# CrawlScript/tf_geometric

Measured on NVIDIA H100. Metric: edges/sec GCN+GAT fwd on 2.4M-node/123M-edge synthetic; %HBM roofline, higher is better.
Workload: dtype f32

## Files before the change

### tf_geometric_b200/csrc/gemm_proj.cu

```cuda
#include "common.cuh"
#include <type_traits>

namespace tfgk {
namespace proj {

constexpr int BM = 128;
constexpr int BK = 32;
constexpr int kUN = 128;
constexpr int kThreads = 256;
constexpr int kApitch = BK + 4;
constexpr int kStageBytes = BM * kApitch * 4;
constexpr int kMaxBlocks = 4;
constexpr int kMaxParts = 8;

struct Params {
    const float *A[kMaxParts];
    int64_t lda, part_rows;
    int first_tile;
    int M, K, kpad, nb, tiles_m, n_groups;
    const float *B[kMaxBlocks]; int64_t ldb[kMaxBlocks];
    const float *bias[kMaxBlocks]; int act[kMaxBlocks]; int ncols[kMaxBlocks]; int transb[kMaxBlocks];
    float *C[kMaxBlocks]; int64_t ldc[kMaxBlocks];
};

struct Plan {
    uint32_t kpad, b_bytes, ring_off, stages, total;
    explicit Plan(int K) {
        kpad = (uint32_t)((K + 7) / 8) * 8;
        b_bytes = (uint32_t)kUN * kpad * 4u;
        ring_off = 2u * b_bytes + kUN * 4u;
        const uint32_t budget = 227u * 1024u;
        stages = 0;
        for (uint32_t st = 4; st >= 2; --st)
            if (ring_off + st * kStageBytes <= budget) { stages = st; break; }
        total = ring_off + stages * kStageBytes;
    }
};

__device__ __forceinline__ uint32_t smem_u32(const void *p) { return (uint32_t)__cvta_generic_to_shared(p); }

__device__ __forceinline__ uint32_t w_offset(int n, int k, int kpad) {
    return (uint32_t)(n >> 3) * (uint32_t)(kpad * 32) + (uint32_t)(k >> 2) * 128u + (uint32_t)(n & 7) * 16u + (uint32_t)(k & 3) * 4u;
}

__device__ __forceinline__ uint64_t make_desc(uint32_t saddr, uint32_t sbo_bytes) {
    uint64_t d = 0;
    d |= (uint64_t)((saddr & 0x3FFFFu) >> 4);
    d |= (uint64_t)(128u >> 4) << 16;
    d |= (uint64_t)(sbo_bytes >> 4) << 32;
    return d;
}

__device__ __forceinline__ void split_tf32(float a, uint32_t &hi, uint32_t &lo) {
    asm("cvt.rna.tf32.f32 %0, %1;" : "=r"(hi) : "f"(a));
    lo = __float_as_uint(a - __uint_as_float(hi));
}

__device__ __forceinline__ void cp_async16_zfill(uint32_t dst, const void *src, uint32_t src_bytes) {
    asm volatile("cp.async.cg.shared.global [%0], [%1], 16, %2;" ::"r"(dst), "l"(src), "r"(src_bytes) : "memory");
}

__device__ __forceinline__ void wgmma_fence() { asm volatile("wgmma.fence.sync.aligned;" ::: "memory"); }
__device__ __forceinline__ void wgmma_commit() { asm volatile("wgmma.commit_group.sync.aligned;" ::: "memory"); }
__device__ __forceinline__ void wgmma_wait_all() { asm volatile("wgmma.wait_group.sync.aligned 0;" ::: "memory"); }

__device__ __forceinline__ void wgmma_m64n128k8(float (&d)[64], const uint32_t (&a)[4], uint64_t b_desc, uint32_t accumulate) {
    asm volatile(
        "{\n\t.reg .pred p;\n\t"
        "setp.ne.b32 p, %69, 0;\n\t"
        "wgmma.mma_async.sync.aligned.m64n128k8.f32.tf32.tf32 "
        "{%0, %1, %2, %3, %4, %5, %6, %7, %8, %9, %10, %11, %12, %13, %14, %15, "
        "%16, %17, %18, %19, %20, %21, %22, %23, %24, %25, %26, %27, %28, %29, %30, %31, "
        "%32, %33, %34, %35, %36, %37, %38, %39, %40, %41, %42, %43, %44, %45, %46, %47, "
        "%48, %49, %50, %51, %52, %53, %54, %55, %56, %57, %58, %59, %60, %61, %62, %63}, "
        "{%64, %65, %66, %67}, %68, p, 1, 1;\n\t}"
        : "+f"(d[0]), "+f"(d[1]), "+f"(d[2]), "+f"(d[3]), "+f"(d[4]), "+f"(d[5]), "+f"(d[6]), "+f"(d[7]),
          "+f"(d[8]), "+f"(d[9]), "+f"(d[10]), "+f"(d[11]), "+f"(d[12]), "+f"(d[13]), "+f"(d[14]), "+f"(d[15]),
          "+f"(d[16]), "+f"(d[17]), "+f"(d[18]), "+f"(d[19]), "+f"(d[20]), "+f"(d[21]), "+f"(d[22]), "+f"(d[23]),
          "+f"(d[24]), "+f"(d[25]), "+f"(d[26]), "+f"(d[27]), "+f"(d[28]), "+f"(d[29]), "+f"(d[30]), "+f"(d[31]),
          "+f"(d[32]), "+f"(d[33]), "+f"(d[34]), "+f"(d[35]), "+f"(d[36]), "+f"(d[37]), "+f"(d[38]), "+f"(d[39]),
          "+f"(d[40]), "+f"(d[41]), "+f"(d[42]), "+f"(d[43]), "+f"(d[44]), "+f"(d[45]), "+f"(d[46]), "+f"(d[47]),
          "+f"(d[48]), "+f"(d[49]), "+f"(d[50]), "+f"(d[51]), "+f"(d[52]), "+f"(d[53]), "+f"(d[54]), "+f"(d[55]),
          "+f"(d[56]), "+f"(d[57]), "+f"(d[58]), "+f"(d[59]), "+f"(d[60]), "+f"(d[61]), "+f"(d[62]), "+f"(d[63])
        : "r"(a[0]), "r"(a[1]), "r"(a[2]), "r"(a[3]), "l"(b_desc), "r"(accumulate)
        : "memory");
}

__device__ __forceinline__ int tile_index(const Params &p, int group, int it) {
    int tl = group + it * p.n_groups + p.first_tile;
    return tl >= p.tiles_m ? tl - p.tiles_m : tl;
}

template <int STAGES>
__global__ void __launch_bounds__(kThreads, 1) gemm_proj_kernel(const Params p) {
    extern __shared__ __align__(128) uint8_t smem[];
    const int tid = threadIdx.x, lane = tid & 31, warp = tid >> 5;
    const int cb = blockIdx.x % p.nb, group = blockIdx.x / p.nb;
    const int kpad = p.kpad;
    const uint32_t b_bytes = (uint32_t)kUN * kpad * 4u;
    uint8_t *w_hi = smem, *w_lo = smem + b_bytes;
    float *s_bias = reinterpret_cast<float *>(smem + 2 * b_bytes);
    uint8_t *ring = smem + 2 * b_bytes + kUN * 4;
    const uint32_t ring_addr = smem_u32(ring);

    const int ncols = p.ncols[cb];
    const int my_tiles = group < p.tiles_m ? (p.tiles_m - group + p.n_groups - 1) / p.n_groups : 0;
    const int kb_per_tile = (p.K + BK - 1) / BK;
    const int total = my_tiles * kb_per_tile;

    auto load_stage = [&](int j) {
        if (j < total) {
            const int64_t row0 = (int64_t)tile_index(p, group, j / kb_per_tile) * BM;
            const int part = (int)(row0 / p.part_rows);
            const float *a_tile = p.A[part] + (row0 - (int64_t)part * p.part_rows) * p.lda;
            const int rows = (int)min((int64_t)BM, (int64_t)p.M - row0);
            const int k0 = (j % kb_per_tile) * BK;
            const uint32_t dst0 = ring_addr + (uint32_t)(j % STAGES) * kStageBytes;
            const int ch = tid & 7, gk = k0 + ch * 4;
            const uint32_t bytes = gk < p.K ? (uint32_t)min(16, (p.K - gk) * 4) : 0u;
#pragma unroll
            for (int i = 0; i < (BM * BK / 4) / kThreads; ++i) {
                const int r = (tid >> 3) + i * (kThreads / 8);
                const bool ok = r < rows && bytes != 0;
                cp_async16_zfill(dst0 + (uint32_t)(r * kApitch + ch * 4) * 4u, ok ? a_tile + (int64_t)r * p.lda + gk : p.A[0],
                                 ok ? bytes : 0u);
            }
        }
        asm volatile("cp.async.commit_group;" ::: "memory");
    };

#pragma unroll
    for (int s = 0; s < STAGES - 1; ++s) load_stage(s);

    {
        const float *B = p.B[cb];
        const int64_t ldb = p.ldb[cb];
        const bool tb = p.transb[cb] != 0;
        for (int idx = tid; idx < kUN * kpad; idx += kThreads) {
            int n, k;
            if (tb) { n = idx / kpad; k = idx % kpad; } else { k = idx / kUN; n = idx % kUN; }
            const float w = (n < ncols && k < p.K) ? (tb ? B[(int64_t)n * ldb + k] : B[(int64_t)k * ldb + n]) : 0.0f;
            uint32_t hi, lo;
            split_tf32(w, hi, lo);
            const uint32_t off = w_offset(n, k, kpad);
            *reinterpret_cast<uint32_t *>(w_hi + off) = hi;
            *reinterpret_cast<uint32_t *>(w_lo + off) = lo;
        }
        if (tid < kUN) s_bias[tid] = (p.bias[cb] != nullptr && tid < ncols) ? p.bias[cb][tid] : 0.0f;
    }
    asm volatile("fence.proxy.async.shared::cta;" ::: "memory");
    __syncthreads();

    const uint32_t w_hi_addr = smem_u32(w_hi), w_lo_addr = smem_u32(w_lo), sbo = (uint32_t)kpad * 32u;
    const int frag_row = (warp >> 2) * 64 + (warp & 3) * 16 + (lane >> 2);
    const int frag_col = lane & 3;
    const int act = p.act[cb];
    float *C = p.C[cb];
    const int64_t ldc = p.ldc[cb];
    const bool vec2 = (ldc % 2) == 0 && (reinterpret_cast<uintptr_t>(C) & 7u) == 0;
    float acc[64];
#pragma unroll
    for (int i = 0; i < 64; ++i) acc[i] = 0.0f;

    uint32_t ah[2][BK / 8][4], al[2][BK / 8][4];
    auto stage = [&](auto parity, int j) {
        constexpr int P = decltype(parity)::value;
        asm volatile("cp.async.wait_group %0;" ::"n"(STAGES - 2) : "memory");
        __syncthreads();
        load_stage(j + STAGES - 1);
        const int kb = j % kb_per_tile;
        const float *As = reinterpret_cast<const float *>(ring + (size_t)(j % STAGES) * kStageBytes);
#pragma unroll
        for (int ks = 0; ks < BK / 8; ++ks) {
            const float *a_r0 = As + frag_row * kApitch + ks * 8 + frag_col;
            const float *a_r8 = a_r0 + 8 * kApitch;
            split_tf32(a_r0[0], ah[P][ks][0], al[P][ks][0]);
            split_tf32(a_r8[0], ah[P][ks][1], al[P][ks][1]);
            split_tf32(a_r0[4], ah[P][ks][2], al[P][ks][2]);
            split_tf32(a_r8[4], ah[P][ks][3], al[P][ks][3]);
        }
        wgmma_wait_all();
        wgmma_fence();
#pragma unroll
        for (int ks = 0; ks < BK / 8; ++ks) {
            const int kg = kb * BK + ks * 8;
            if (kg < kpad) {
                const uint32_t koff = (uint32_t)(kg >> 2) * 128u;
                const uint64_t dh = make_desc(w_hi_addr + koff, sbo), dl = make_desc(w_lo_addr + koff, sbo);
                wgmma_m64n128k8(acc, al[P][ks], dh, (kb | ks) != 0);
                wgmma_m64n128k8(acc, ah[P][ks], dl, 1u);
                wgmma_m64n128k8(acc, ah[P][ks], dh, 1u);
            }
        }
        wgmma_commit();
        if (kb == kb_per_tile - 1) {
            wgmma_wait_all();
            const int64_t row0 = (int64_t)tile_index(p, group, j / kb_per_tile) * BM + frag_row;
#pragma unroll
            for (int h = 0; h < 2; ++h) {
                const int64_t row = row0 + 8 * h;
                if (row < p.M) {
                    float *crow = C + row * ldc;
#pragma unroll
                    for (int nb8 = 0; nb8 < kUN / 8; ++nb8) {
                        const int col = nb8 * 8 + 2 * frag_col;
                        const float v0 = apply_act(acc[4 * nb8 + 2 * h] + s_bias[col], act);
                        const float v1 = apply_act(acc[4 * nb8 + 2 * h + 1] + s_bias[col + 1], act);
                        if (vec2 && col + 1 < ncols) {
                            *reinterpret_cast<float2 *>(crow + col) = make_float2(v0, v1);
                        } else {
                            if (col < ncols) crow[col] = v0;
                            if (col + 1 < ncols) crow[col + 1] = v1;
                        }
                    }
                }
            }
        }
    };
    for (int j = 0; j < total; j += 2) {
        stage(std::integral_constant<int, 0>(), j);
        if (j + 1 < total) stage(std::integral_constant<int, 1>(), j + 1);
    }
    wgmma_wait_all();
    asm volatile("cp.async.wait_group 0;" ::: "memory");
}

template <int STAGES>
static int launch(const Params &p, int grid, uint32_t smem_bytes, cudaStream_t st) {
    TFGK_CUDA(ensure_dynamic_smem(gemm_proj_kernel<STAGES>, smem_bytes));
    gemm_proj_kernel<STAGES><<<grid, kThreads, smem_bytes, st>>>(p);
    TFGK_LAUNCH_CHECK();
    return TFGK_OK;
}

}
}

using namespace tfgk;

extern "C" int tfgk_gemm_proj_f32(const float *const *A_parts, int32_t n_parts, int64_t part_rows, int64_t lda,
                                  int32_t M, int32_t K, const tfgk_proj_block *blocks, int32_t n_blocks,
                                  int32_t first_part, int32_t max_ctas, void *stream) {
    TFGK_CHECK_ARG(A_parts != nullptr && blocks != nullptr, "gemm_proj: null argument");
    TFGK_CHECK_ARG(n_parts >= 1 && n_parts <= proj::kMaxParts, "gemm_proj: n_parts=%d not in [1, %d]", n_parts, proj::kMaxParts);
    TFGK_CHECK_ARG(n_blocks >= 1 && n_blocks <= proj::kMaxBlocks, "gemm_proj: n_blocks=%d not in [1, %d]", n_blocks, proj::kMaxBlocks);
    TFGK_CHECK_ARG(M >= 0 && K >= 1, "gemm_proj: bad size (M=%d, K=%d)", M, K);
    TFGK_CHECK_ARG(first_part >= 0 && first_part < n_parts, "gemm_proj: first_part=%d out of range", first_part);
    if (M == 0) return TFGK_OK;
    if (n_parts > 1)
        TFGK_CHECK_ARG(part_rows > 0 && part_rows % proj::BM == 0 && (int64_t)n_parts * part_rows >= M,
                       "gemm_proj: part_rows=%lld must be a positive multiple of %d covering M=%d", (long long)part_rows, proj::BM, M);
    if (K > 512 || (lda % 4) != 0 || lda < K) return TFGK_ERR_UNSUPPORTED;
    proj::Params p;
    for (int i = 0; i < proj::kMaxParts; ++i) {
        p.A[i] = A_parts[i < n_parts ? i : 0];
        if (!aligned16(p.A[i]) || p.A[i] == nullptr) return i < n_parts && A_parts[i] == nullptr
            ? set_error(TFGK_ERR_INVALID_ARGUMENT, "gemm_proj: A part %d is null", i) : TFGK_ERR_UNSUPPORTED;
    }
    p.lda = lda; p.part_rows = n_parts > 1 ? part_rows : (int64_t)1 << 40;
    p.M = M; p.K = K; p.nb = n_blocks;
    p.tiles_m = (int)ceil_div64(M, proj::BM);
    p.first_tile = n_parts > 1 ? (int)((int64_t)first_part * part_rows / proj::BM) : 0;
    if (p.first_tile >= p.tiles_m) p.first_tile = 0;
    for (int b = 0; b < proj::kMaxBlocks; ++b) {
        const tfgk_proj_block &blk = blocks[b < n_blocks ? b : 0];
        if (b < n_blocks) {
            TFGK_CHECK_ARG(blk.B != nullptr && blk.C != nullptr, "gemm_proj: block %d has a null operand", b);
            TFGK_CHECK_ARG(blk.ncols >= 1 && blk.ldb >= (blk.transB ? K : blk.ncols) && blk.ldc >= blk.ncols,
                           "gemm_proj: block %d has bad sizes", b);
            TFGK_CHECK_ARG(blk.act == TFGK_ACT_NONE || blk.act == TFGK_ACT_RELU, "gemm_proj: unknown activation %d", blk.act);
            if (blk.ncols > proj::kUN) return TFGK_ERR_UNSUPPORTED;
        }
        p.B[b] = blk.B; p.ldb[b] = blk.ldb; p.bias[b] = blk.bias; p.act[b] = blk.act; p.ncols[b] = blk.ncols;
        p.transb[b] = blk.transB;
        p.C[b] = blk.C; p.ldc[b] = blk.ldc;
    }
    const proj::Plan L(K);
    if (L.stages == 0) return TFGK_ERR_UNSUPPORTED;
    p.kpad = (int)L.kpad;
    int dev = 0, sms = 0;
    TFGK_CUDA(cudaGetDevice(&dev));
    TFGK_CUDA(cudaDeviceGetAttribute(&sms, cudaDevAttrMultiProcessorCount, dev));
    if (max_ctas > 0 && max_ctas < sms) sms = max_ctas;
    int n_groups = sms / n_blocks;
    if (n_groups < 1) n_groups = 1;
    if (n_groups > p.tiles_m) n_groups = p.tiles_m;
    p.n_groups = n_groups;
    const int grid = n_groups * n_blocks;
    cudaStream_t st = as_stream(stream);
    if (L.stages >= 4) return proj::launch<4>(p, grid, L.total, st);
    if (L.stages == 3) return proj::launch<3>(p, grid, L.total, st);
    return proj::launch<2>(p, grid, L.total, st);
}
```

Measured before the change: 3.067 billion.

## Add warp-specialized bulk-copy projection GEMM with mbarrier ring and two consumer warpgroups

Result: no change. 3.129 billion, median of 6 (+2.0%).

```diff
diff --git a/tf_geometric_b200/csrc/gemm_proj.cu b/tf_geometric_b200/csrc/gemm_proj.cu
--- a/tf_geometric_b200/csrc/gemm_proj.cu
+++ b/tf_geometric_b200/csrc/gemm_proj.cu
@@ -63,6 +63,7 @@
 __device__ __forceinline__ void wgmma_fence() { asm volatile("wgmma.fence.sync.aligned;" ::: "memory"); }
 __device__ __forceinline__ void wgmma_commit() { asm volatile("wgmma.commit_group.sync.aligned;" ::: "memory"); }
 __device__ __forceinline__ void wgmma_wait_all() { asm volatile("wgmma.wait_group.sync.aligned 0;" ::: "memory"); }
+__device__ __forceinline__ void wgmma_wait_one() { asm volatile("wgmma.wait_group.sync.aligned 1;" ::: "memory"); }
 
 __device__ __forceinline__ void wgmma_m64n128k8(float (&d)[64], const uint32_t (&a)[4], uint64_t b_desc, uint32_t accumulate) {
     asm volatile(
@@ -233,6 +234,188 @@
     return TFGK_OK;
 }
 
+constexpr int kWsRows = 64;
+constexpr int kWsThreads = 288;
+constexpr int kWsProducerWarp = 8;
+
+struct WsPlan {
+    uint32_t kpad, pitch, stage_bytes, ring_off, stages, total;
+    explicit WsPlan(int K) {
+        kpad = (uint32_t)((K + 7) / 8) * 8;
+        pitch = kpad + 4;
+        stage_bytes = (uint32_t)kWsRows * pitch * 4u;
+        ring_off = 2u * (uint32_t)kUN * kpad * 4u + kUN * 4u;
+        const uint32_t budget = 227u * 1024u;
+        stages = 0;
+        for (uint32_t st = 4; st >= 2; --st)
+            if (ring_off + st * (stage_bytes + 16u) <= budget) { stages = st; break; }
+        total = ring_off + stages * (stage_bytes + 16u);
+    }
+};
+
+__device__ __forceinline__ void mbar_wait(uint32_t bar, uint32_t parity) {
+    uint32_t done = 0;
+    for (uint32_t spin = 0; !done; ++spin) {
+        asm volatile(
+            "{\n\t.reg .pred p;\n\t"
+            "mbarrier.try_wait.parity.shared::cta.b64 p, [%1], %2;\n\t"
+            "selp.u32 %0, 1, 0, p;\n\t}"
+            : "=r"(done) : "r"(bar), "r"(parity) : "memory");
+        if (spin > (1u << 28)) __trap();
+    }
+}
+
+template <int S>
+__global__ void __launch_bounds__(kWsThreads, 1) gemm_proj_ws_kernel(const Params p, const uint32_t pitch) {
+    extern __shared__ __align__(128) uint8_t smem[];
+    const int tid = threadIdx.x, lane = tid & 31, warp = __shfl_sync(0xffffffffu, tid >> 5, 0);
+    const int cb = blockIdx.x % p.nb, group = blockIdx.x / p.nb;
+    const int kpad = p.kpad;
+    const uint32_t b_bytes = (uint32_t)kUN * kpad * 4u, stage_bytes = (uint32_t)kWsRows * pitch * 4u;
+    uint8_t *w_hi = smem, *w_lo = smem + b_bytes;
+    float *s_bias = reinterpret_cast<float *>(smem + 2 * b_bytes);
+    uint8_t *ring = smem + 2 * b_bytes + kUN * 4;
+    const uint32_t ring_addr = smem_u32(ring);
+    const uint32_t full0 = ring_addr + (uint32_t)S * stage_bytes, empty0 = full0 + 8u * S;
+    const int ncols = p.ncols[cb];
+    const int my_tiles = group < p.tiles_m ? (p.tiles_m - group + p.n_groups - 1) / p.n_groups : 0;
+
+    if (tid == 0) {
+#pragma unroll
+        for (int s = 0; s < S; ++s) {
+            asm volatile("mbarrier.init.shared::cta.b64 [%0], 1;" ::"r"(full0 + 8u * s));
+            asm volatile("mbarrier.init.shared::cta.b64 [%0], %1;" ::"r"(empty0 + 8u * s), "r"(kWsRows * 2));
+        }
+        asm volatile("fence.mbarrier_init.release.cluster;" ::: "memory");
+    }
+    {
+        const float *B = p.B[cb];
+        const int64_t ldb = p.ldb[cb];
+        const bool tb = p.transb[cb] != 0;
+        for (int idx = tid; idx < kUN * kpad; idx += kWsThreads) {
+            int n, k;
+            if (tb) { n = idx / kpad; k = idx % kpad; } else { k = idx / kUN; n = idx % kUN; }
+            const float w = (n < ncols && k < p.K) ? (tb ? B[(int64_t)n * ldb + k] : B[(int64_t)k * ldb + n]) : 0.0f;
+            uint32_t hi, lo;
+            split_tf32(w, hi, lo);
+            const uint32_t off = w_offset(n, k, kpad);
+            *reinterpret_cast<uint32_t *>(w_hi + off) = hi;
+            *reinterpret_cast<uint32_t *>(w_lo + off) = lo;
+        }
+        if (tid < kUN) s_bias[tid] = (p.bias[cb] != nullptr && tid < ncols) ? p.bias[cb][tid] : 0.0f;
+    }
+    asm volatile("fence.proxy.async.shared::cta;" ::: "memory");
+    __syncthreads();
+
+    if (warp == kWsProducerWarp) {
+        for (int r = lane; r < S * kWsRows; r += 32)
+            for (int k = p.K; k < kpad; ++k) reinterpret_cast<float *>(ring)[r * (int)pitch + k] = 0.0f;
+        __syncwarp();
+        const uint32_t row_bytes = (uint32_t)p.K * 4u;
+        for (int i = 0; i < my_tiles; ++i) {
+            const int s = i % S;
+            if (i >= S) mbar_wait(empty0 + 8u * s, (uint32_t)((i / S) - 1) & 1u);
+            const int64_t row0 = (int64_t)(group + i * p.n_groups) * kWsRows;
+            const int rows = (int)min((int64_t)kWsRows, (int64_t)p.M - row0);
+            const uint32_t full = full0 + 8u * s, dst = ring_addr + (uint32_t)s * stage_bytes;
+            if (lane == 0)
+                asm volatile("mbarrier.arrive.expect_tx.shared::cta.b64 _, [%0], %1;" ::"r"(full), "r"((uint32_t)rows * row_bytes)
+                             : "memory");
+            __syncwarp();
+            for (int r = lane; r < rows; r += 32)
+                asm volatile("cp.async.bulk.shared::cluster.global.mbarrier::complete_tx::bytes [%0], [%1], %2, [%3];"
+                             ::"r"(dst + (uint32_t)r * pitch * 4u), "l"(p.A[0] + (row0 + r) * p.lda), "r"(row_bytes), "r"(full)
+                             : "memory");
+        }
+        return;
+    }
+
+    const int wg = warp >> 2;
+    const uint32_t w_hi_addr = smem_u32(w_hi), w_lo_addr = smem_u32(w_lo), sbo = (uint32_t)kpad * 32u;
+    const int frag_row = (warp & 3) * 16 + (lane >> 2);
+    const int frag_col = lane & 3;
+    const int act = p.act[cb];
+    float *C = p.C[cb];
+    const int64_t ldc = p.ldc[cb];
+    const bool vec2 = (ldc % 2) == 0 && (reinterpret_cast<uintptr_t>(C) & 7u) == 0;
+    float acc[64];
+#pragma unroll
+    for (int i = 0; i < 64; ++i) acc[i] = 0.0f;
+
+    const int n_chunks = (p.K + BK - 1) / BK;
+    const int total = (my_tiles - wg + 1) / 2 * n_chunks;
+    uint32_t ah[2][BK / 8][4], al[2][BK / 8][4];
+    auto stage = [&](auto parity, int j) {
+        constexpr int P = decltype(parity)::value;
+        const int kb = j % n_chunks, i = wg + 2 * (j / n_chunks), s = i % S;
+        if (kb == 0) mbar_wait(full0 + 8u * s, (uint32_t)(i / S) & 1u);
+        const float *As = reinterpret_cast<const float *>(ring + (size_t)s * stage_bytes);
+        float av[BK / 8][4];
+#pragma unroll
+        for (int ks = 0; ks < BK / 8; ++ks) {
+            const float *a_r0 = As + frag_row * (int)pitch + min(kb * BK + ks * 8, kpad - 8) + frag_col;
+            const float *a_r8 = a_r0 + 8 * (int)pitch;
+            av[ks][0] = a_r0[0]; av[ks][1] = a_r8[0]; av[ks][2] = a_r0[4]; av[ks][3] = a_r8[4];
+        }
+        wgmma_wait_one();
+#pragma unroll
+        for (int ks = 0; ks < BK / 8; ++ks)
+#pragma unroll
+            for (int e = 0; e < 4; ++e) split_tf32(av[ks][e], ah[P][ks][e], al[P][ks][e]);
+        if (kb == 0 && i > 0) asm volatile("bar.sync %0, %1;" ::"r"(1 + wg), "n"(2 * 128) : "memory");
+        wgmma_fence();
+#pragma unroll
+        for (int ks = 0; ks < BK / 8; ++ks) {
+            const int kg = kb * BK + ks * 8;
+            if (kg < kpad) {
+                const uint32_t koff = (uint32_t)(kg >> 2) * 128u;
+                const uint64_t dh = make_desc(w_hi_addr + koff, sbo), dl = make_desc(w_lo_addr + koff, sbo);
+                wgmma_m64n128k8(acc, al[P][ks], dh, (kb | ks) != 0);
+                wgmma_m64n128k8(acc, ah[P][ks], dl, 1u);
+                wgmma_m64n128k8(acc, ah[P][ks], dh, 1u);
+            }
+        }
+        wgmma_commit();
+        if (kb == n_chunks - 1) {
+            asm volatile("mbarrier.arrive.shared::cta.b64 _, [%0];" ::"r"(empty0 + 8u * s) : "memory");
+            if (i + 1 < my_tiles) asm volatile("bar.arrive %0, %1;" ::"r"(1 + (wg ^ 1)), "n"(2 * 128) : "memory");
+            wgmma_wait_all();
+            const int64_t row0 = (int64_t)(group + i * p.n_groups) * kWsRows + frag_row;
+#pragma unroll
+            for (int h = 0; h < 2; ++h) {
+                const int64_t row = row0 + 8 * h;
+                if (row < p.M) {
+                    float *crow = C + row * ldc;
+#pragma unroll
+                    for (int nb8 = 0; nb8 < kUN / 8; ++nb8) {
+                        const int col = nb8 * 8 + 2 * frag_col;
+                        const float v0 = apply_act(acc[4 * nb8 + 2 * h] + s_bias[col], act);
+                        const float v1 = apply_act(acc[4 * nb8 + 2 * h + 1] + s_bias[col + 1], act);
+                        if (vec2 && col + 1 < ncols) {
+                            *reinterpret_cast<float2 *>(crow + col) = make_float2(v0, v1);
+                        } else {
+                            if (col < ncols) crow[col] = v0;
+                            if (col + 1 < ncols) crow[col + 1] = v1;
+                        }
+                    }
+                }
+            }
+        }
+    };
+    for (int j = 0; j < total; j += 2) {
+        stage(std::integral_constant<int, 0>(), j);
+        if (j + 1 < total) stage(std::integral_constant<int, 1>(), j + 1);
+    }
+}
+
+template <int S>
+static int launch_ws(const Params &p, uint32_t pitch, int grid, uint32_t smem_bytes, cudaStream_t st) {
+    TFGK_CUDA(ensure_dynamic_smem(gemm_proj_ws_kernel<S>, smem_bytes));
+    gemm_proj_ws_kernel<S><<<grid, kWsThreads, smem_bytes, st>>>(p, pitch);
+    TFGK_LAUNCH_CHECK();
+    return TFGK_OK;
+}
+
 }
 }
 
@@ -282,12 +465,26 @@
     TFGK_CUDA(cudaGetDevice(&dev));
     TFGK_CUDA(cudaDeviceGetAttribute(&sms, cudaDevAttrMultiProcessorCount, dev));
     if (max_ctas > 0 && max_ctas < sms) sms = max_ctas;
-    int n_groups = sms / n_blocks;
-    if (n_groups < 1) n_groups = 1;
-    if (n_groups > p.tiles_m) n_groups = p.tiles_m;
-    p.n_groups = n_groups;
-    const int grid = n_groups * n_blocks;
     cudaStream_t st = as_stream(stream);
+    auto groups_for = [&](int tiles_m) {
+        int n_groups = sms / n_blocks;
+        if (n_groups < 1) n_groups = 1;
+        return n_groups > tiles_m ? tiles_m : n_groups;
+    };
+
+    const char *impl = getenv("TFGK_PROJ_IMPL");
+    const proj::WsPlan WS(K);
+    if (!(impl != nullptr && impl[0] == 'r') && n_parts == 1 && K % 4 == 0 && WS.stages >= 2) {
+        p.tiles_m = (int)ceil_div64(M, proj::kWsRows);
+        p.n_groups = groups_for(p.tiles_m);
+        const int grid = p.n_groups * n_blocks;
+        if (WS.stages >= 4) return proj::launch_ws<4>(p, WS.pitch, grid, WS.total, st);
+        if (WS.stages == 3) return proj::launch_ws<3>(p, WS.pitch, grid, WS.total, st);
+        return proj::launch_ws<2>(p, WS.pitch, grid, WS.total, st);
+    }
+
+    p.n_groups = groups_for(p.tiles_m);
+    const int grid = p.n_groups * n_blocks;
     if (L.stages >= 4) return proj::launch<4>(p, grid, L.total, st);
     if (L.stages == 3) return proj::launch<3>(p, grid, L.total, st);
     return proj::launch<2>(p, grid, L.total, st);
```
